# Dimev/grail-rs

Measured on AMD Instinct MI355X. Metric: audio samples/sec (whole node) at 48 kHz, batch=65536 utterances, higher is better.
Workload: dtype f32

## Files before the change

### grail-rs_amd/csrc/api_internal.hpp

```cpp
#pragma once

#include <dlfcn.h>
#include <hip/hip_runtime.h>
#include <rccl/rccl.h>

#include <algorithm>
#include <atomic>
#include <cmath>
#include <condition_variable>
#include <cstdio>
#include <deque>
#include <map>
#include <memory>
#include <mutex>
#include <thread>
#include <cstdlib>
#include <cstring>
#include <new>
#include <string>
#include <type_traits>
#include <unordered_map>
#include <utility>
#include <vector>

#include "../../include/grail_hip.h"
#include "division_window.h"
#include "dyn_plan.h"
#include "fir_plan.h"
#include "iir_plan.h"
#include "kernels.h"
#include "limit_plan.h"
#include "meter_plan.h"
#include "resample_plan.h"


#ifdef GRAIL_FAST_PROF
constexpr size_t TRUNCATED_WORDS = 8 + 64;
#else
constexpr size_t TRUNCATED_WORDS = 4;
#endif

struct Options {
    int64_t fast_option = 0;
    int64_t fast_limit = (int64_t)GRAIL_FAST_SHARPNESS_LIMIT;
    int64_t mid_option = 1;
    int64_t mid_limit = (int64_t)GRAIL_FAST_SHARPNESS_LIMIT_EXACT_COEFFICIENTS;
    int64_t lanes_option = 0;
    int64_t skip_silent_option = 1;
    int64_t pipeline_option = 1;
    int64_t pipe_round32 = 1;
    int64_t pipe_spread = 1;
    int64_t pipe4_max_groups = -1;
    int64_t pipe8_max_groups = -1;
    int64_t scan_option = 1;
    int64_t scan_max_utts = -1;
    int64_t scan_split_max = -1;
    int64_t scan_debug = 0;
    int64_t split_option = 1;
    int64_t split_chunks = 0;
    int64_t split_span = 0;
    int64_t split_ff_permille = 165;
    int64_t split_min_utts = -1;
    int64_t composite_option = 1;
    int64_t row_groups_option = 1;
    int64_t ragged_option = 1;
    int64_t two_waves_option = 1;
    int64_t packed_option = 1;
    int64_t sort_option = 1;
};

struct VoiceInfo {
    bool upper_silent = false, live4_ok = false, scan_ok = false, split_ok = false;
    uint32_t warmup = 0;
};

struct VoiceFacts {
    std::vector<VoiceInfo> voice_info;
    bool voices_upper_silent = false;
    bool voices_live4_ok = false;
    bool voices_scan_ok = false;
    bool voices_split_ok = false;
    uint32_t max_warmup = 0;
    float max_rate = 0.0f;
    float max_dt = 0.0f;
    float max_pitch_jitter = 0.0f;
    double voices_sharpness = INFINITY;
    std::vector<double> voice_sharpness;
};

struct LaunchStats {
    std::string last_kernel = "none";
    int last_formants = 8, last_lanes = 0, last_pipe = 0;
    int last_split = 0;
    int last_fast = 0;
    int last_blocks = 0;
    int last_packed = 0;
    uint64_t slow_steps = 0;
    uint64_t fast_tiles = 0, general_steps = 0;
};

namespace grail {
namespace host {

int fail(int status, const std::string &msg);
int hip_fail(hipError_t e, const char *what);
std::string &last_error();

#define HIP_TRY(expr)                                  \
    do {                                               \
        hipError_t e_ = (expr);                        \
        if (e_ != hipSuccess) return ::grail::host::hip_fail(e_, #expr); \
    } while (0)

template <typename H, hipError_t (*Release)(H)>
class Handle {
public:
    Handle() = default;
    Handle(Handle &&o) noexcept : h_(std::exchange(o.h_, H{})) {}
    Handle &operator=(Handle &&o) noexcept
    {
        if (this != &o) {
            reset();
            h_ = std::exchange(o.h_, H{});
        }
        return *this;
    }
    ~Handle() { reset(); }
    H get() const { return h_; }
    void reset()
    {
        if (h_) (void)Release(h_);
        h_ = H{};
    }
    template <typename Make>
    hipError_t renew(Make make)
    {
        reset();
        const hipError_t e = make(&h_);
        if (e != hipSuccess) h_ = H{};
        return e;
    }

private:
    H h_{};
};

struct Event : Handle<hipEvent_t, hipEventDestroy> {
    hipError_t create(bool timing = false)
    {
        return renew([&](hipEvent_t *ev) { return timing ? hipEventCreate(ev) : hipEventCreateWithFlags(ev, hipEventDisableTiming); });
    }
    operator hipEvent_t() const { return get(); }
};

struct Stream : Handle<hipStream_t, hipStreamDestroy> {
    hipError_t create()
    {
        return renew([](hipStream_t *s) { return hipStreamCreateWithFlags(s, hipStreamNonBlocking); });
    }
    operator hipStream_t() const { return get(); }
};

template <typename T>
class DeviceBuffer {
public:
    T *get() const { return static_cast<T *>(mem_.get()); }
    size_t capacity() const { return mem_.get() ? cap_ : 0; }
    void reset() { mem_.reset(); }
    hipError_t alloc(size_t n)
    {
        cap_ = std::max<size_t>(n, 1);
        return mem_.renew([&](void **p) { return hipMalloc(p, cap_ * sizeof(T)); });
    }
    int reserve(hipStream_t stream, size_t need, size_t want)
    {
        if (capacity() >= std::max<size_t>(need, 1)) return GRAIL_OK;
        if (get()) HIP_TRY(hipStreamSynchronize(stream));
        HIP_TRY(alloc(want));
        return GRAIL_OK;
    }
    int reserve(hipStream_t stream, size_t need) { return reserve(stream, need, need); }

private:
    Handle<void *, hipFree> mem_;
    size_t cap_ = 0;
};

template <typename Tp>
hipError_t upload(DeviceBuffer<Tp> &dst, const void *src, size_t count, hipStream_t stream)
{
    const hipError_t e = dst.alloc(count);
    if (e != hipSuccess || !src || !count) return e;
    return hipMemcpyAsync(dst.get(), src, count * sizeof(Tp), hipMemcpyHostToDevice, stream);
}

struct RowIndex {
    std::vector<uint32_t> host;
    DeviceBuffer<uint32_t> dev;
    hipError_t fill(const uint32_t *given, uint32_t n_rows, bool own_row, hipStream_t stream)
    {
        host.resize(n_rows);
        for (uint32_t u = 0; u < n_rows; ++u) host[u] = given ? given[u] : (own_row ? u : 0u);
        return upload(dev, host.data(), n_rows, stream);
    }
};

class PinnedBuffer {
public:
    void *get() const { return mem_.get(); }
    size_t capacity() const { return mem_.get() ? cap_ : 0; }
    void reset() { mem_.reset(); }
    hipError_t alloc(size_t bytes)
    {
        cap_ = bytes;
        return mem_.renew([&](void **p) { return hipHostMalloc(p, bytes, hipHostMallocDefault); });
    }

private:
    Handle<void *, hipHostFree> mem_;
    size_t cap_ = 0;
};

struct Family {
    int L = 1;
    uint32_t pipe = 0;
    uint32_t live4 = 0;
    bool half = false;
    uint32_t fast = 0;
    int split_k = 0;
    uint32_t split_bounds[SPLIT_MAX_CHUNKS + 1] = {};
    uint32_t split_active = 0;
    bool scan = false;
    uint32_t scan_pipe = 0;
};

struct Block {
    uint32_t rows;
    Family f;
};

struct PlanCache {
    uint64_t key[6] = {};
    std::vector<Block> plan;
};

}
}

struct PlanEnv {
    int cus = 256;
    Options opt;
    VoiceFacts facts;
    uint64_t voices_epoch = 0;
};

struct CtxPart {
    virtual ~CtxPart() = default;
};

struct grail_ctx : PlanEnv {
    int device = 0;
    int device_cus = 256;
    grail::host::Stream stream;
    grail::host::Event ev_start, ev_stop;
    bool have_timing = false;
    uint64_t options_epoch = 0;
    std::vector<grail_voice> voices;
    grail::host::DeviceBuffer<grail::DevVoice> d_voices;
    grail::host::DeviceBuffer<float> d_voice_elems;
    LaunchStats stats;
    grail::host::DeviceBuffer<uint32_t> d_truncated;
    uint32_t seen_counters[4] = {0, 0, 0, 0};
    ncclComm_t comm = nullptr;
    uint32_t comm_rank = 0, comm_world = 1;
    std::unique_ptr<CtxPart> host_pipe;
    std::unique_ptr<CtxPart> mix_state;
    std::unique_ptr<CtxPart> level_state;
    std::unique_ptr<CtxPart> transform_state;
};

struct grail_stream {
    const grail_batch *batch = nullptr;
    grail::host::DeviceBuffer<uint32_t> d_state;
    uint64_t lanes = 0;
    int L = 1;
    bool started = false;
    bool live4 = false, half_capable = false, any_blend = false;
    uint64_t voices_epoch = 0;
    std::unique_ptr<grail_batch> own;
    uint32_t ring_cap = 0;
    grail::host::DeviceBuffer<uint32_t> d_counts;
    grail::host::DeviceBuffer<uint32_t> d_open;
    grail::host::DeviceBuffer<uint32_t> d_consumed;
    std::vector<uint32_t> appended;
    std::vector<uint32_t> consumed;
    std::vector<uint8_t> open;
    std::vector<grail_synthesis_elem> last_elem;
    std::vector<uint8_t> last_has;
    grail::host::DeviceBuffer<grail::DevSeg> d_new;
    grail::host::DeviceBuffer<float> d_new_elems;
    grail::host::DeviceBuffer<uint32_t> d_new_offs;
    grail::host::PinnedBuffer h_stage[2];
    grail::host::Event ev_stage[2];
    bool stage_busy[2] = {false, false};
    int stage_next = 0;
};

struct grail_fir {
    uint32_t n_filters = 0;
    uint32_t tail_max = 0;
    std::vector<double> image;
    std::vector<uint32_t> desc;
    grail::host::DeviceBuffer<double> d_taps;
    grail::host::DeviceBuffer<uint32_t> d_desc;
    uint32_t taps_max = 0;
};

struct ChunkedStream {
    uint32_t n_rows = 0;
    uint32_t units = 0;
    uint32_t ring_cap = 0;
    grail::host::DeviceBuffer<uint64_t> d_state;
    grail::host::DeviceBuffer<float> d_ring;
    std::vector<uint8_t> mark;
    grail::host::DeviceBuffer<uint8_t> d_mark;
    grail::host::Event ev_mark;
};

struct grail_filter_stream : ChunkedStream {
    const grail_fir *set = nullptr;
    grail::host::RowIndex filter;
};

struct grail_resample_stream : ChunkedStream {
    uint32_t up = 0, down = 0, taps = 0;
    std::vector<int32_t> table;
    grail::host::DeviceBuffer<int32_t> d_table;
};

struct grail_limit_stream : ChunkedStream {
    uint32_t group = 1;
    float ceiling = 0.0f;
    uint32_t ell = 0;
};

struct grail_meter_stream : ChunkedStream {
    uint32_t sample_rate = 0, hop = 0;
    uint64_t max_hops = 0;
    double coef[10] = {};
    grail::host::DeviceBuffer<double> d_ledger;
};

struct grail_iir {
    uint32_t n_filters = 0;
    uint32_t bound = 1;
    std::vector<double> image;
    std::vector<uint32_t> sections;
    grail::host::DeviceBuffer<double> d_image;
    grail::host::DeviceBuffer<uint32_t> d_sections;
    std::vector<double> block_image;
    grail::host::DeviceBuffer<double> d_block;
};

struct grail_iir_stream : ChunkedStream {
    const grail_iir *set = nullptr;
    uint32_t tail = 0;
    grail::host::RowIndex filter;
};

struct grail_dyn {
    uint32_t n_curves = 0;
    std::vector<double> image;
    std::vector<double> alpha;
    std::vector<uint32_t> detector;
    grail::host::DeviceBuffer<double> d_image;
    grail::host::DeviceBuffer<double> d_alpha;
    grail::host::DeviceBuffer<uint32_t> d_detector;
};

struct grail_dyn_stream : ChunkedStream {
    const grail_dyn *set = nullptr;
    uint32_t n_keys = 0;
    grail::host::RowIndex curve;
    grail::host::RowIndex key_row;
};

struct BatchFacts {
    uint32_t n_utt = 0;
    uint32_t n_segs = 0;
    uint32_t max_voice_id = 0;
    bool phoneme_mode = true;
    bool any_blend = false;
    bool plain = false;
    float max_seconds = 0.0f;
    float min_length = 0.0f;
    float min_pitch = 0.0f;
    uint64_t len_bound_epoch = 0;
    bool len_bound_known = false;
    double elems_sharpness = 0.0;
    uint32_t elems_warmup = 0;
    uint64_t elems_warmup_epoch = 0;
    bool elems_live4_ok = false;
    bool elems_scan_ok = false;
    std::vector<uint32_t> used_voices;
    std::vector<float> granule_samples;
    std::vector<uint32_t> granule_segs, granule_kinks;
};

struct RowGroup : BatchFacts {
    uint32_t slot0 = 0;
    mutable grail::host::PlanCache plan_cache;
};

struct PackedPerm {
    uint32_t view = 0;
    uint32_t slot0 = 0, rows = 0, per_block = 0, cus = 0;
    uint32_t family = 0;
    grail::host::DeviceBuffer<uint32_t> d_perm;
    double model_ms = 0.0, plain_ms = 0.0;
};

struct grail_batch : BatchFacts {
    grail::host::DeviceBuffer<grail::DevSeg> d_segs;
    grail::host::DeviceBuffer<uint32_t> d_offsets, d_voice_ids, d_seeds;
    grail::host::DeviceBuffer<uint32_t> d_perm;
    std::vector<uint32_t> perm_host;
    grail::host::DeviceBuffer<uint32_t> d_len_bound;
    grail::host::DeviceBuffer<float> d_elems;
    std::vector<RowGroup> groups;
    uint64_t groups_epoch = 0;
    mutable std::mutex lock;
    mutable grail::host::PlanCache plan_cache;
    mutable std::vector<PackedPerm> packed;
};
static_assert(!std::is_copy_constructible_v<grail_batch>, "a batch owns its device arrays: row groups are BatchFacts, not batches");

#include "launch_plan.h"

namespace grail {
namespace host {

int bind(grail_ctx *ctx);
int bind_device(grail_ctx *ctx, const char *who);

void name_voices(BatchFacts &b, const uint32_t *voice_ids, uint32_t n_utt);
bool blend_is_pow2(float blend_length);
int check_offsets(const uint32_t *seg_offsets, uint32_t n_utt, uint32_t *n_segs);
int install_voices(grail_ctx *ctx, const grail_voice *voices, uint32_t n_voices);
int check_ready(grail_ctx *ctx, const grail_batch *batch);

bool live4_ok(const grail_voice &v);
bool live4_elems_ok(const grail_synthesis_elem *elems, size_t n_elems, float jitter_delta_formant_frequency);
bool scan_voice_ok(const grail_voice &v);
bool scan_elems_ok(const grail_synthesis_elem *elems, size_t n_elems, float jitter_delta_formant_frequency);
uint32_t voice_warmup(const grail_voice &v);
uint32_t elems_warmup(const grail_synthesis_elem *elems, size_t n_elems, double jitter_delta_formant_frequency);
double elems_sharpness(const grail_synthesis_elem *elems, size_t n);
double batch_sharpness(const PlanEnv *ctx, const BatchFacts *batch);
int fast_tier_for(const PlanEnv *ctx, const BatchFacts *batch, int arithmetic);
int fast_tier(const PlanEnv *ctx, const BatchFacts *batch);
bool split_grid(uint32_t span, uint32_t warmup, int K, double r, uint32_t *b);

void batch_args(const grail_ctx *ctx, const grail_batch *batch, uint32_t row0, SynthArgs &a);
int synthesize_rows(grail_ctx *ctx, const grail_batch *batch, float *out_dev, int16_t *out_pcm16_dev, uint64_t out_stride,
                    uint32_t *out_len_dev, uint32_t first = 0, uint32_t count = 0, uint32_t family_rows = 0);

void comm_release(grail_ctx *ctx);
int drop_batch(grail_ctx *ctx, grail_batch *batch, int rc);
int level_block_gains(grail_ctx *ctx, int mode, uint32_t sample_rate, const float *rows_dev, uint64_t row_stride,
                      const uint32_t *len_dev, const uint32_t *row_len, uint32_t n_rows, const uint32_t *item_rows,
                      const float *item_level_db, uint32_t n_items, float *gains, uint32_t *n_unleveled,
                      const float *ceiling_db, uint32_t *n_limited);
uint32_t level_table_rate(const grail_ctx *ctx);
int say_segments(const std::vector<grail_voice> &voices, const char *const *texts_utf8, uint32_t n_texts,
                 const uint32_t *voice_ids, std::vector<grail_phoneme_elem> &segs, std::vector<uint32_t> &offs);
int comm_init_all(grail_ctx *const *ctxs, const int *devices, uint32_t n);

}
}
```

### grail-rs_amd/csrc/family_cost.cpp

```cpp
#include "api_internal.hpp"

#include <functional>
#include <queue>

using namespace grail;
using namespace grail::host;

namespace grail {
namespace host {

double batch_span(const PlanEnv *ctx, const BatchFacts *batch, uint64_t out_stride)
{
    double span = std::ceil((double)batch->max_seconds * ctx->facts.max_rate) + 64.0;
    if (!(span >= 64.0)) span = 64.0;
    return std::fmin(span, (double)(out_stride ? out_stride : 1));
}

constexpr double MID_MS_4 = 32.6, MID_MS_8 = 57.2;
static double lane_ms_per_sample(bool fast, bool live4, int L)
{
    static const double exact4[4] = {40.6, 26.9, 16.3, 18.2}, exact8[4] = {77.1, 43.5, 25.8, 15.7};
    static const double fast4[4] = {15.5, 13.6, 12.8, 12.1}, fast8[4] = {23.6, 16.4, 13.3, 12.0};
    const int i = L == 1 ? 0 : L == 2 ? 1 : L == 4 ? 2 : 3;
    return (fast ? (live4 ? fast4 : fast8) : (live4 ? exact4 : exact8))[i] / 96006.0;
// ... 61 lines not shown
    const bool nfa4 = f.live4 != 0;
    const int li = f.L == 1 ? 0 : f.L == 2 ? 1 : f.L == 4 ? 2 : 3;
    if (!f.fast) {
        const double T = (f.L == 1 || (!nfa4 && f.L == 4)) ? 32.0 : 64.0;
        const double tiles = std::fmax(samples / T, 1.0);
        const double event_tiles = tiles * (1.0 - std::exp(-segs / tiles));
        const double runs = f.L == 1 ? 1.0 : f.L == 2 ? (nfa4 ? 0.74 : 0.60) : f.L == 4 ? (nfa4 ? 0.51 : 1.0) : 0.58;
        return samples * lane_ms_per_sample(false, nfa4, f.L) + event_tiles * (nfa4 ? 0.007 : 0.008) * (T / 32.0) * runs +
               (f.L == 1 ? segs * (nfa4 ? 0.0015 : 0.0037) : 0.0);
    }
    static const double m4[4] = {1.16, 1.10, 1.06, 1.02}, c4[4] = {0.00475, 0.0050, 0.00675, 0.00925};
    static const double m8[4] = {1.08, 1.06, 1.04, 1.02}, c8[4] = {0.00775, 0.00675, 0.0070, 0.0095};
    const double events = segs + kinks;
    const double density = events / ((64.0 / (double)f.L) * std::fmax(samples, 1.0));
    const double m = 1.0 + ((nfa4 ? m4 : m8)[li] - 1.0) * std::fmin(1.0, density / 3.0e-4);
    const double rate = f.fast == 2u ? mid_ms_per_sample(nfa4) : lane_ms_per_sample(true, nfa4, f.L);
    return samples * rate * m + events * (nfa4 ? c4 : c8)[li];
}

struct WaveRows {
    double samples = 0.0, segs = 0.0, kinks = 0.0;
};
static WaveRows wave_rows(const BatchFacts *batch, size_t g, size_t per_wave, size_t g1)
{
    WaveRows w;
    for (size_t k = g; k < std::min(g + per_wave, g1); ++k) {
        w.samples = std::fmax(w.samples, (double)batch->granule_samples[k]);
        w.segs += batch->granule_segs[k];
        w.kinks += batch->granule_kinks[k];
    }
    return w;
}
double ragged_wave_cost(const BatchFacts *batch, const Family &f, size_t g, size_t per_wave, size_t g1, double span)
{
    const WaveRows w = wave_rows(batch, g, per_wave, g1);
    return ragged_wave_ms(f, std::fmin(w.samples + 64.0, span), w.segs, w.kinks);
}
static double mean_samples(const BatchFacts *batch, const GranuleRange &r)
{
    double mean = 0.0;
    for (size_t g = r.g0; g < r.g1; ++g) mean += (double)batch->granule_samples[g];
    return mean / (double)(r.g1 - r.g0);
}

static double ragged_scan_cost(const PlanEnv *ctx, const BatchFacts *batch, const Family &f, const GranuleRange &r, uint32_t rows,
                               double span)
{
    return std::fmax(family_cost(ctx, f, rows, std::fmin(mean_samples(batch, r) + 64.0, span)),
                     family_cost(ctx, f, 1u, std::fmin(span, (double)batch->granule_samples[r.g0] + 64.0)));
}

static double ragged_pipe_cost(const PlanEnv *ctx, const BatchFacts *batch, const Family &f, const GranuleRange &r, uint32_t rows,
                               double span)
{
    const size_t g0 = r.g0, g1 = r.g1;
    double longest = std::fmin(span, std::fmax((double)batch->granule_samples[g0], 0.0) + 64.0);
    if (std::ceil((double)rows / (f.live4 ? 16.0 : 8.0)) > (double)ctx->cus)
        longest = 0.55 * longest + 0.45 * std::fmin(longest, mean_samples(batch, r) + 64.0);
    double c = family_cost(ctx, f, rows, longest);
    c *= 1.15;
    double segs = batch->granule_segs[g0];
    if (f.live4 && g0 + 1 < g1) segs += batch->granule_segs[g0 + 1];
    const uint32_t fill = pipe_fill_for(ctx, batch, f, rows);
    if (fill) segs *= (double)fill / (f.live4 ? 16.0 : 8.0);
    const double rounds = std::fmax(longest / 32.0, 1.0);
    const double groups = std::ceil((double)rows / (f.live4 ? 16.0 : 8.0));
    c += 0.011 * rounds * (1.0 - std::exp(-segs / rounds)) * std::ceil(groups / ((f.pipe == 2 ? 1.0 : 2.0) * (double)ctx->cus));
    return c;
}

static double ragged_split_cost(const PlanEnv *ctx, const BatchFacts *batch, const Family &f, const GranuleRange &r, uint32_t rows)
{
    const WaveRows w = wave_rows(batch, r.g0, 8, r.g1);
    const double len = std::fmax((double)batch->granule_samples[r.g0], 64.0), part = (double)f.split_bounds[1] / len;
    Family lane = f;
    lane.split_k = 0;
    lane.L = 1;
    return split_rounds(ctx, f, rows) * (1.2 * ragged_wave_ms(lane, (double)f.split_bounds[1], w.segs * part, w.kinks * part) + 0.12);
}

static double two_wave_cost(const PlanEnv *ctx, const BatchFacts *batch, const Family &f, const GranuleRange &r, double span)
{
    const size_t g0 = r.g0, g1 = r.g1, per_wave = granules_per_wave(f);
    const uint64_t simds = ctx_simds(ctx);
    struct Simd { double t, a, b; };
    auto take = [](Simd &m, const double w) {
        if (m.b < 0.0) m.b = w;
        else if (w <= m.b) m.a = w;
        else { m.a = m.b; m.b = w; }
    };
    double ev_sum = 0.0, lane_samples = 0.0;
    for (size_t g = g0; g < g1; ++g) {
        ev_sum += (double)batch->granule_segs[g] + (double)batch->granule_kinks[g];
        lane_samples += 8.0 * std::fmax((double)batch->granule_samples[g], 1.0);
    }
    const double pace2 = 1.0 / (2.0 * cohabit_gain(f, ev_sum / std::fmax(lane_samples, 1.0)));
    std::vector<Simd> sm(simds, Simd{0.0, -1.0, -1.0});
    auto next_done = [&](const Simd &m) {
        return m.a < 0.0 ? m.t + m.b : m.t + m.a / pace2;
    };
    typedef std::pair<double, size_t> Ev;
    std::priority_queue<Ev, std::vector<Ev>, std::greater<Ev>> done_at;
    const size_t n_waves = (g1 - g0 + per_wave - 1) / per_wave;
    const bool fold = n_waves > simds && n_waves <= 2 * simds;
    size_t g = g0, filled = 0;
    for (; g < g1 && filled < 2 * simds; g += per_wave, ++filled)
        take(sm[filled % simds], ragged_wave_cost(batch, f, fold && filled >= simds ? g0 + (n_waves - 1 - (filled - simds)) * per_wave : g,
                                                  per_wave, g1, span));
    for (size_t i = 0; i < simds; ++i)
        if (sm[i].b >= 0.0) done_at.push(Ev(next_done(sm[i]), i));
    double makespan = 0.0;
    while (!done_at.empty()) {
        const Ev ev = done_at.top();
        done_at.pop();
        Simd &m = sm[ev.second];
        if (m.a < 0.0) {
            m.t += m.b;
            m.b = -1.0;
        } else {
            m.t += m.a / pace2;
            m.b -= m.a;
            m.a = -1.0;
        }
        makespan = std::fmax(makespan, m.t);
        if (g < g1) {
            take(m, ragged_wave_cost(batch, f, g, per_wave, g1, span));
            g += per_wave;
        }
        if (m.b >= 0.0) done_at.push(Ev(next_done(m), ev.second));
    }
    const double waves = std::ceil((double)(g1 - g0) / (double)per_wave);
    const double scale = !f.fast ? (f.L == 2 ? 0.84 : 0.91) : (f.L == 2 && waves > 2.0 * (double)simds ? 1.15 : 1.0);
    return makespan * scale;
}

static double dispatched_cost(const PlanEnv *ctx, const BatchFacts *batch, const Family &f, uint32_t slot0, uint32_t rows, double span)
{
    double plain_ms = 0.0, packed_ms = 0.0;
    const bool packed = packed_launch_order(ctx, batch, f, slot0, rows, span, nullptr, nullptr, &plain_ms, &packed_ms);
    return 0.96 * (packed ? packed_ms : plain_ms);
}

double ragged_cost(const PlanEnv *ctx, const BatchFacts *batch, const Family &f, uint32_t slot0, uint32_t rows, double span)
{
    if (batch->granule_samples.empty() || rows == 0) return family_cost(ctx, f, rows, span);
    const GranuleRange r = granule_range(batch, slot0, rows);
    if (f.scan) return ragged_scan_cost(ctx, batch, f, r, rows, span);
    if (f.pipe) return ragged_pipe_cost(ctx, batch, f, r, rows, span);
    if (f.split_k) return ragged_split_cost(ctx, batch, f, r, rows);
    if (family_cohabits(ctx, f, rows)) return two_wave_cost(ctx, batch, f, r, span);
    return dispatched_cost(ctx, batch, f, slot0, rows, span);
}

}
}
```

### grail-rs_amd/csrc/grail_api.cpp

```cpp
#include "api_internal.hpp"

using namespace grail;
using namespace grail::host;

static_assert(sizeof(grail_synthesis_elem) == 196, "SynthesisElem is 49 x f32");
static_assert(sizeof(grail_phoneme_elem) == sizeof(DevSeg), "PhonemeElem uploads as-is");
static_assert(offsetof(grail_phoneme_elem, phoneme) == offsetof(DevSeg, elem), "layout");
static_assert(offsetof(grail_phoneme_elem, frequency) == offsetof(DevSeg, frequency), "layout");
static_assert(sizeof(grail_voice) == 4 + 2 * 196 + 5 * 4, "Voice layout");
static_assert(GRAIL_UNIQUE_ID_BYTES == NCCL_UNIQUE_ID_BYTES, "unique id size");

namespace grail {
namespace host {

namespace {
thread_local std::string g_last_error;
std::atomic<uint64_t> g_epoch{0};
}

std::string &last_error() { return g_last_error; }

int fail(int status, const std::string &msg)
{
    g_last_error = msg;
// ... 207 lines not shown
    b.used_voices.assign(voice_ids, voice_ids + n_utt);
    std::sort(b.used_voices.begin(), b.used_voices.end());
    b.used_voices.erase(std::unique(b.used_voices.begin(), b.used_voices.end()), b.used_voices.end());
    b.max_voice_id = b.used_voices.back();
}

int upload_common(grail_ctx *ctx, grail_batch *b, const uint32_t *seg_offsets,
                  const uint32_t *voice_ids, const uint32_t *jitter_seeds, uint32_t n_utt)
{
    HIP_TRY(upload(b->d_offsets, seg_offsets, (size_t)n_utt + 1, ctx->stream));
    name_voices(*b, voice_ids, n_utt);
    if (voice_ids) HIP_TRY(upload(b->d_voice_ids, voice_ids, n_utt, ctx->stream));
    if (jitter_seeds) HIP_TRY(upload(b->d_seeds, jitter_seeds, n_utt, ctx->stream));
    b->n_utt = n_utt;
    HIP_TRY(hipStreamSynchronize(ctx->stream));
    return GRAIL_OK;
}

int install_voices(grail_ctx *ctx, const grail_voice *voices, uint32_t n_voices)
{
    if (!voices || n_voices == 0) return fail(GRAIL_ERR_INVALID_ARG, "no voices given");
    std::vector<DevVoice> dv(n_voices);
    std::vector<float> elems((size_t)n_voices * NUM_VOICED * ELEM_FLOATS);
    for (uint32_t v = 0; v < n_voices; ++v) {
        dv[v].sample_rate = voices[v].sample_rate;
        dv[v].jitter_frequency = voices[v].jitter_frequency;
        dv[v].jitter_delta_frequency = voices[v].jitter_delta_frequency;
        dv[v].jitter_delta_formant_frequency = voices[v].jitter_delta_formant_frequency;
        dv[v].jitter_delta_amplitude = voices[v].jitter_delta_amplitude;
        dv[v].elem_base = v * NUM_VOICED;
        dv[v].warmup = voice_warmup(voices[v]);
        dv[v].pad = 0;
        std::memcpy(&elems[(size_t)v * NUM_VOICED * ELEM_FLOATS], voices[v].phonemes,
                    sizeof(grail_synthesis_elem) * NUM_VOICED);
    }
    HIP_TRY(hipStreamSynchronize(ctx->stream));
    ctx->voices.clear();
    HIP_TRY(upload(ctx->d_voices, dv.data(), dv.size(), ctx->stream));
    HIP_TRY(upload(ctx->d_voice_elems, elems.data(), elems.size(), ctx->stream));
    HIP_TRY(hipStreamSynchronize(ctx->stream));
    VoiceFacts facts;
    facts.voices_upper_silent = facts.voices_live4_ok = facts.voices_scan_ok = facts.voices_split_ok = true;
    facts.voices_sharpness = 0.0;
    facts.voice_info.resize(n_voices);
    facts.voice_sharpness.resize(n_voices);
    for (uint32_t v = 0; v < n_voices; ++v) {
        VoiceInfo &vi = facts.voice_info[v];
        vi.upper_silent = true;
        for (int p = 0; p < NUM_VOICED; ++p)
            for (int i = NF / 2; i < NF; ++i) {
                uint32_t bits;
                std::memcpy(&bits, &voices[v].phonemes[p].formant_amp[i], sizeof bits);
                vi.upper_silent = vi.upper_silent && bits == 0u;
            }
        vi.live4_ok = live4_ok(voices[v]);
        vi.scan_ok = scan_voice_ok(voices[v]);
        vi.warmup = dv[v].warmup;
        vi.split_ok = dv[v].warmup != 0u && voices[v].sample_rate > 0.0f && std::isfinite(voices[v].sample_rate);
        facts.voices_upper_silent = facts.voices_upper_silent && vi.upper_silent;
        facts.voices_live4_ok = facts.voices_live4_ok && vi.live4_ok;
        facts.voices_scan_ok = facts.voices_scan_ok && vi.scan_ok;
        facts.voices_split_ok = facts.voices_split_ok && vi.split_ok;
        if (vi.warmup > facts.max_warmup) facts.max_warmup = vi.warmup;
        if (voices[v].sample_rate > facts.max_rate) facts.max_rate = voices[v].sample_rate;
        const float dt = 1.0f / voices[v].sample_rate;
        if (!(dt <= facts.max_dt)) facts.max_dt = dt;
        const float pj = std::fabs(voices[v].jitter_delta_frequency);
        if (!(pj <= facts.max_pitch_jitter)) facts.max_pitch_jitter = pj;
        facts.voice_sharpness[v] = elems_sharpness(voices[v].phonemes, NUM_VOICED);
        facts.voices_sharpness = std::fmax(facts.voices_sharpness, facts.voice_sharpness[v]);
    }
    ctx->voices.assign(voices, voices + n_voices);
    ctx->voices_epoch = ++g_epoch;
    ctx->facts = std::move(facts);
    return GRAIL_OK;
}

int check_ready(grail_ctx *ctx, const grail_batch *batch)
{
    if (!batch) return fail(GRAIL_ERR_INVALID_ARG, "batch is NULL");
    if (ctx->voices.empty() || !ctx->d_voices.get() || !ctx->d_voice_elems.get())
        return fail(GRAIL_ERR_NO_VOICES, "call grail_set_voices first");
    if (batch->max_voice_id >= ctx->voices.size())
        return fail(GRAIL_ERR_INVALID_ARG, "a voice id exceeds the voice table");
    return GRAIL_OK;
}

}
}

extern "C" {

int grail_abi_version(void) { return GRAIL_ABI_VERSION; }

const char *grail_status_string(int status)
{
    switch (status) {
    case GRAIL_OK: return "ok";
    case GRAIL_ERR_INVALID_ARG: return "invalid argument";
    case GRAIL_ERR_NO_DEVICE: return "no usable HIP device (there is no CPU fallback)";
    case GRAIL_ERR_HIP: return "HIP runtime error";
    case GRAIL_ERR_BUFFER_TOO_SMALL: return "an utterance did not end within out_stride samples";
    case GRAIL_ERR_OUT_OF_MEMORY: return "out of device memory";
    case GRAIL_ERR_RCCL: return "RCCL error";
    case GRAIL_ERR_NO_VOICES: return "no voice table set";
    default: return "unknown status";
    }
}

const char *grail_last_error(void) { return g_last_error.c_str(); }

int grail_device_count(int *count)
{
    if (!count) return fail(GRAIL_ERR_INVALID_ARG, "count is NULL");
    *count = 0;
    int n = 0;
    hipError_t e = hipGetDeviceCount(&n);
    if (e != hipSuccess) return hip_fail(e, "hipGetDeviceCount");
    *count = n;
    return GRAIL_OK;
}

int grail_device_pci_bus_id(grail_ctx *ctx, char *out, size_t cap)
{
    if (!ctx || !out || cap < 16) return fail(GRAIL_ERR_INVALID_ARG, "grail_device_pci_bus_id: NULL argument or cap < 16");
    out[0] = 0;
    HIP_TRY(hipDeviceGetPCIBusId(out, (int)cap, ctx->device));
    return GRAIL_OK;
}

int grail_create(int device, grail_ctx **out)
{
    if (!out) return fail(GRAIL_ERR_INVALID_ARG, "out is NULL");
    *out = nullptr;
    int n = 0;
    hipError_t e = hipGetDeviceCount(&n);
    if (e != hipSuccess || n <= 0)
        return fail(GRAIL_ERR_NO_DEVICE,
                    std::string("no HIP device: ") + (e != hipSuccess ? hipGetErrorString(e) : "count 0"));
    if (device < 0 || device >= n) return fail(GRAIL_ERR_NO_DEVICE, "device index out of range");
    HIP_TRY(hipSetDevice(device));
    hipDeviceProp_t prop;
    HIP_TRY(hipGetDeviceProperties(&prop, device));
    if (std::strncmp(prop.gcnArchName, "gfx950", 6) != 0)
        return fail(GRAIL_ERR_NO_DEVICE, std::string("device ") + std::to_string(device) + " is " + prop.gcnArchName +
                                             ": this library holds gfx950 (MI355X) kernels only");
    if (prop.multiProcessorCount <= 0) return fail(GRAIL_ERR_NO_DEVICE, "the device reports no compute units");
    std::unique_ptr<grail_ctx> ctx(new (std::nothrow) grail_ctx());
    if (!ctx) return fail(GRAIL_ERR_OUT_OF_MEMORY, "host allocation failed");
    ctx->device = device;
    ctx->cus = ctx->device_cus = prop.multiProcessorCount;
    hipError_t err;
    if ((err = ctx->stream.create()) != hipSuccess ||
        (err = ctx->ev_start.create(true)) != hipSuccess ||
        (err = ctx->ev_stop.create(true)) != hipSuccess ||
        (err = ctx->d_truncated.alloc(TRUNCATED_WORDS)) != hipSuccess ||
        (err = hipMemsetAsync(ctx->d_truncated.get(), 0, TRUNCATED_WORDS * sizeof(uint32_t), ctx->stream)) != hipSuccess ||
        (err = hipStreamSynchronize(ctx->stream)) != hipSuccess)
        return hip_fail(err, "grail_create");
    *out = ctx.release();
    return GRAIL_OK;
}

int grail_destroy(grail_ctx *ctx)
{
    if (!ctx) return GRAIL_OK;
    (void)hipSetDevice(ctx->device);
    if (ctx->stream) (void)hipStreamSynchronize(ctx->stream);
    comm_release(ctx);
    delete ctx;
    return GRAIL_OK;
}

int grail_set_voices(grail_ctx *ctx, const grail_voice *voices, uint32_t n_voices)
{
    int rc = bind(ctx);
    if (rc) return rc;
    return install_voices(ctx, voices, n_voices);
}

int grail_get_voices(grail_ctx *ctx, grail_voice *voices, uint32_t cap, uint32_t *n_voices)
{
    if (!ctx) return fail(GRAIL_ERR_INVALID_ARG, "ctx is NULL");
    if (n_voices) *n_voices = (uint32_t)ctx->voices.size();
    if (voices)
        for (uint32_t i = 0; i < cap && i < ctx->voices.size(); ++i) voices[i] = ctx->voices[i];
    return GRAIL_OK;
}

uint64_t grail_length_bound(const float *segment_lengths, uint32_t n_segments, float sample_rate)
{
    if (!(sample_rate > 0.0f) || (n_segments && !segment_lengths)) return UINT64_MAX;
    const double dt = (double)(1.0f / sample_rate);
    double samples = 0.0;
    for (uint32_t i = 0; i < n_segments; ++i) {
        if (!std::isfinite(segment_lengths[i])) return UINT64_MAX;
        samples += segment_bound(segment_lengths[i], dt);
    }
    return samples < 1.8e19 ? (uint64_t)samples : UINT64_MAX;
}

int grail_batch_upload(grail_ctx *ctx, const grail_phoneme_elem *segs, const uint32_t *seg_offsets,
                       const uint32_t *voice_ids, const uint32_t *jitter_seeds, uint32_t n_utt,
                       grail_batch **out)
{
    int rc = bind(ctx);
    if (rc) return rc;
    if (!out) return fail(GRAIL_ERR_INVALID_ARG, "out is NULL");
    *out = nullptr;
    uint32_t n_segs = 0;
    if ((rc = check_offsets(seg_offsets, n_utt, &n_segs))) return rc;
    if (n_segs && !segs) return fail(GRAIL_ERR_INVALID_ARG, "segs is NULL");
    for (uint32_t i = 0; i < n_segs; ++i)
        if (segs[i].phoneme < 0 || segs[i].phoneme >= GRAIL_PH_COUNT)
            return fail(GRAIL_ERR_INVALID_ARG, "phoneme discriminant out of range");
    std::unique_ptr<grail_batch> b(new (std::nothrow) grail_batch());
    if (!b) return fail(GRAIL_ERR_OUT_OF_MEMORY, "host allocation failed");
    b->phoneme_mode = true;
    b->n_segs = n_segs;
    const std::vector<RowStats> rows = batch_stats(ctx, b.get(), segs, seg_offsets, n_utt,
                                                   [](float f) { return std::fmin(f, 0.5f); });
    HIP_TRY(upload(b->d_segs, segs, n_segs, ctx->stream));
    if ((rc = upload_common(ctx, b.get(), seg_offsets, voice_ids, jitter_seeds, n_utt)) ||
        (rc = upload_len_bound(ctx, b.get(), rows, n_utt)) || (rc = upload_length_order(ctx, b.get(), rows, n_utt)))
        return rc;
    *out = b.release();
    return GRAIL_OK;
}

int grail_batch_upload_elems(grail_ctx *ctx, const grail_sequence_elem *segs,
                             const uint32_t *seg_offsets, const uint32_t *voice_ids,
                             const uint32_t *jitter_seeds, uint32_t n_utt, grail_batch **out)
{
    int rc = bind(ctx);
    if (rc) return rc;
    if (!out) return fail(GRAIL_ERR_INVALID_ARG, "out is NULL");
    *out = nullptr;
    uint32_t n_segs = 0;
    if ((rc = check_offsets(seg_offsets, n_utt, &n_segs))) return rc;
    if (n_segs && !segs) return fail(GRAIL_ERR_INVALID_ARG, "segs is NULL");
    std::vector<DevSeg> ds(n_segs);
    std::vector<float> elems((size_t)(n_segs ? n_segs : 1) * ELEM_FLOATS);
    for (uint32_t i = 0; i < n_segs; ++i) {
        ds[i].elem = segs[i].has_elem ? (int32_t)i : -1;
        ds[i].length = segs[i].length;
        ds[i].blend_length = segs[i].blend_length;
        ds[i].frequency = segs[i].elem.frequency;
        std::memcpy(&elems[(size_t)i * ELEM_FLOATS], &segs[i].elem, sizeof(grail_synthesis_elem));
    }
    std::unique_ptr<grail_batch> b(new (std::nothrow) grail_batch());
    if (!b) return fail(GRAIL_ERR_OUT_OF_MEMORY, "host allocation failed");
    b->phoneme_mode = false;
    b->n_segs = n_segs;
    const std::vector<RowStats> rows = batch_stats(ctx, b.get(), ds.data(), seg_offsets, n_utt, [](float f) { return f; });
    struct FormantsHash {
        size_t operator()(const float *p) const
        {
            uint64_t h = 0x9E3779B97F4A7C15ull, w;
            for (int i = 0; i < 24; ++i) {
                std::memcpy(&w, p + 1 + 2 * i, sizeof w);
                h = (h ^ w) * 0xFF51AFD7ED558CCDull;
                h ^= h >> 29;
            }
            return (size_t)h;
        }
    };
    struct FormantsEq {
        bool operator()(const float *a, const float *c) const { return std::memcmp(a + 1, c + 1, 48 * sizeof(float)) == 0; }
    };
    std::unordered_map<const float *, uint32_t, FormantsHash, FormantsEq> ids;
    std::vector<grail_synthesis_elem> distinct;
    std::vector<uint32_t> id_of(n_segs, 0xFFFFFFFFu);
    for (uint32_t i = 0; i < n_segs; ++i) {
        if (!segs[i].has_elem) continue;
        const auto it = ids.emplace((const float *)&segs[i].elem, (uint32_t)distinct.size());
        if (it.second) distinct.push_back(segs[i].elem);
        id_of[i] = it.first->second;
    }
    std::unordered_map<uint64_t, double> pair_sharpness;
    for (uint32_t u = 0; u < n_utt; ++u)
        for (uint32_t i = seg_offsets[u]; i < seg_offsets[u + 1]; ++i) {
            if (!segs[i].has_elem) continue;
            const uint32_t a = id_of[i];
            const uint32_t c = (i + 1 < seg_offsets[u + 1] && segs[i + 1].has_elem) ? id_of[i + 1] : a;
            const uint64_t key = ((uint64_t)std::min(a, c) << 32) | std::max(a, c);
            auto it = pair_sharpness.find(key);
            if (it == pair_sharpness.end()) {
                const grail_synthesis_elem pair[2] = {distinct[a], distinct[c]};
                it = pair_sharpness.emplace(key, elems_sharpness(pair, a == c ? 1 : 2)).first;
            }
            b->elems_sharpness = std::fmax(b->elems_sharpness, it->second);
        }
    HIP_TRY(upload(b->d_segs, ds.data(), n_segs, ctx->stream));
    HIP_TRY(upload(b->d_elems, elems.data(), elems.size(), ctx->stream));
    if ((rc = upload_common(ctx, b.get(), seg_offsets, voice_ids, jitter_seeds, n_utt)) ||
        (rc = upload_len_bound(ctx, b.get(), rows, n_utt)) || (rc = upload_length_order(ctx, b.get(), rows, n_utt)))
        return rc;
    if (!ctx->voices.empty() && b->max_voice_id < ctx->voices.size()) {
        double jd = 0.0;
        bool rates_ok = true;
        for (const uint32_t v : b->used_voices) {
            jd = std::fmax(jd, std::fabs((double)ctx->voices[v].jitter_delta_formant_frequency));
            rates_ok = rates_ok && ctx->voices[v].sample_rate > 0.0f && std::isfinite(ctx->voices[v].sample_rate);
        }
        bool voices4 = true;
        for (const uint32_t v : b->used_voices) {
            grail_voice scalars = ctx->voices[v];
            for (int ph = 0; ph < NUM_VOICED; ++ph) grail_elem_silent(&scalars.phonemes[ph]);
            voices4 = voices4 && live4_ok(scalars);
        }
        b->elems_live4_ok = voices4 && live4_elems_ok(distinct.data(), distinct.size(), (float)jd);
        b->elems_warmup = rates_ok ? elems_warmup(distinct.data(), distinct.size(), jd) : 0u;
        float max_pitch = 0.0f;
        for (uint32_t i = 0; i < n_segs; ++i) max_pitch = std::fmax(max_pitch, segs[i].elem.frequency);
        b->elems_scan_ok = rates_ok && max_pitch <= 0.5f && scan_elems_ok(distinct.data(), distinct.size(), (float)jd);
        b->elems_warmup_epoch = ctx->voices_epoch;
        for (RowGroup &g : b->groups) {
            g.elems_warmup = b->elems_warmup;
            g.elems_warmup_epoch = b->elems_warmup_epoch;
            g.elems_live4_ok = b->elems_live4_ok;
            g.elems_scan_ok = b->elems_scan_ok;
// ... 203 lines not shown
```

### grail-rs_amd/csrc/synthesize.cpp

```cpp
#include "api_internal.hpp"

using namespace grail;
using namespace grail::host;

namespace grail {
namespace host {

struct View {
    const BatchFacts *facts;
    PlanCache *cache;
    uint32_t id, slot0;
};

void batch_args(const grail_ctx *ctx, const grail_batch *batch, uint32_t row0, SynthArgs &a)
{
    a.segs = batch->d_segs.get();
    a.seg_offsets = batch->d_offsets.get() + row0;
    a.voice_ids = batch->d_voice_ids.get() ? batch->d_voice_ids.get() + row0 : nullptr;
    a.seeds = batch->d_seeds.get() ? batch->d_seeds.get() + row0 : nullptr;
    a.elems = batch->phoneme_mode ? ctx->d_voice_elems.get() : batch->d_elems.get();
    a.voices = ctx->d_voices.get();
    a.truncated = ctx->d_truncated.get();
    a.n_voices = (uint32_t)ctx->voices.size();
    a.phoneme_mode = batch->phoneme_mode ? 1u : 0u;
    a.skip_silent = ctx->opt.skip_silent_option ? 1u : 0u;
}

static const uint32_t *packed_perm_of(grail_ctx *ctx, const grail_batch *root, const View &view, const Family &f,
                                      uint64_t out_stride, uint32_t slot0, uint32_t count, int *rc)
{
    *rc = GRAIL_OK;
    if (!ctx->opt.packed_option || root->perm_host.size() < (size_t)slot0 + count) return nullptr;
    const uint32_t family = (uint32_t)f.L | f.fast << 8 | f.live4 << 16;
    std::lock_guard<std::mutex> hold(root->lock);
    for (const PackedPerm &pp : root->packed)
        if (pp.view == view.id && pp.slot0 == slot0 && pp.rows == count && pp.family == family && pp.cus == (uint32_t)ctx->cus)
            return pp.d_perm.get();
    if (root->packed.size() >= 8) return nullptr;
    PackedPerm pp;
    pp.view = view.id;
    pp.slot0 = slot0;
    pp.rows = count;
    pp.family = family;
    pp.cus = (uint32_t)ctx->cus;
    std::vector<uint32_t> order;
    if (packed_launch_order(ctx, view.facts, f, slot0 - view.slot0, count, batch_span(ctx, view.facts, out_stride), &order,
                            &pp.per_block, &pp.plain_ms, &pp.model_ms)) {
        std::vector<uint32_t> perm(count);
        const uint32_t *src = root->perm_host.data() + slot0;
        size_t at = 0;
        for (const uint32_t b : order) {
            const size_t lo = (size_t)b * pp.per_block, hi = std::min<size_t>(lo + pp.per_block, count);
            for (size_t i = lo; i < hi; ++i) perm[at++] = src[i];
        }
        hipError_t e = at == count ? upload(pp.d_perm, perm.data(), count, ctx->stream) : hipErrorInvalidValue;
        if (e == hipSuccess) e = hipStreamSynchronize(ctx->stream);
        if (e != hipSuccess) {
            *rc = hip_fail(e, "packed launch order");
            return nullptr;
        }
    }
    root->packed.push_back(std::move(pp));
    return root->packed.back().d_perm.get();
}

static int launch_block(grail_ctx *ctx, const grail_batch *root, const View &view, const Family &f, float *out_dev,
                        int16_t *out_pcm16_dev, uint64_t out_stride, uint32_t *out_len_dev, uint32_t first, uint32_t slot0,
                        uint32_t count, bool use_perm)
{
    const BatchFacts *batch = view.facts;
    SynthArgs a{};
    const uint32_t row0 = use_perm ? 0u : first + slot0;
    const uint64_t out_shift = use_perm ? 0ull : (uint64_t)slot0 * out_stride;
    batch_args(ctx, root, row0, a);
    a.out_pcm16 = out_pcm16_dev ? out_pcm16_dev + out_shift : nullptr;
    a.perm = use_perm ? root->d_perm.get() + slot0 : nullptr;
    if (use_perm) {
        int rc = GRAIL_OK;
        const uint32_t *packed = packed_perm_of(ctx, root, view, f, out_stride, slot0, count, &rc);
        if (rc) return rc;
        if (packed) {
            a.perm = packed;
            ++ctx->stats.last_packed;
        }
    }
    a.out = out_dev ? out_dev + out_shift : nullptr;
    a.out_len = out_len_dev ? out_len_dev + (use_perm ? 0u : slot0) : nullptr;
    a.out_stride = out_stride;
    a.cap = out_stride;
    a.n_utt = count;
    a.half_capable = batch_half_capable(ctx, batch) ? 1u : 0u;
    a.any_blend = batch->any_blend ? 1u : 0u;
    a.live4 = f.live4;
    a.fast = f.fast;
    a.cohabit = family_cohabits(ctx, f, count) ? 1u : 0u;
    a.len_bound = root->d_len_bound.get() && batch->len_bound_epoch == ctx->voices_epoch ? root->d_len_bound.get() + row0 : nullptr;
    a.pipe_fill = pipe_fill_for(ctx, batch, f, count);
    a.fold_from = 0u;
    if (a.cohabit) {
        const WorkgroupShape wg = workgroup_shape(f);
        const uint32_t blocks = (count + wg.rows - 1u) / wg.rows, round = (uint32_t)ctx_simds(ctx) / wg.waves;
        if (blocks > round && blocks <= 2u * round) a.fold_from = round;
    }
    a.pipe = f.pipe;
    hipError_t e;
    if (f.scan) {
        a.resume = (uint32_t)ctx->opt.scan_debug;
        a.pipe = f.scan_pipe;
        e = launch_scan(a, ctx->stream);
        ctx->stats.last_kernel = a.live4 ? (a.pipe ? "scan_kernel<pairs=2,SPLIT,FAST>" : "scan_kernel<pairs=2,FAST>")
                                   : (a.pipe ? "scan_kernel<pairs=4,SPLIT,FAST>" : "scan_kernel<pairs=4,FAST>");
    } else {
        if (f.split_k) {
            a.split_chunks = (uint32_t)f.split_k;
            a.split_warmup = batch->phoneme_mode ? 0u : batch->elems_warmup;
            std::memcpy(a.split_bounds, f.split_bounds, sizeof a.split_bounds);
        }
        e = launch_synth(a, f.L, ctx->stream);
        ctx->stats.last_kernel = last_kernel_name();
    }
    if (e != hipSuccess) return hip_fail(e, "synth kernel launch");
    return GRAIL_OK;
}

static void record_plan(LaunchStats &st, const Family &f0, size_t n_blocks)
{
    st.last_split = f0.split_k;
    st.last_formants = f0.live4 ? 4 : 8;
    st.last_lanes = f0.scan ? 0 : f0.L;
    st.last_pipe = f0.pipe && !f0.scan ? 1 : 0;
    st.last_packed = 0;
    st.last_fast = 0;
    st.last_blocks = (int)n_blocks;
}

int synthesize_rows(grail_ctx *ctx, const grail_batch *batch, float *out_dev,
                           int16_t *out_pcm16_dev, uint64_t out_stride, uint32_t *out_len_dev,
                           uint32_t first, uint32_t count, uint32_t family_rows)
{
    int rc = bind(ctx);
    if (rc) return rc;
    if ((rc = check_ready(ctx, batch))) return rc;
    if (batch->n_utt == 0) return GRAIL_OK;
    if (!out_dev && !out_pcm16_dev && out_stride) return fail(GRAIL_ERR_INVALID_ARG, "out_dev is NULL");
    if (first > batch->n_utt || count > batch->n_utt - first) return fail(GRAIL_ERR_INVALID_ARG, "row range");
    if (count == 0) count = batch->n_utt - first;
    if (count == 0) return GRAIL_OK;
    const bool use_perm = first == 0 && count == batch->n_utt && batch->d_perm.get();
    auto plan_of = [&](const View &view, const uint32_t rows) {
        const BatchFacts *facts = view.facts;
        std::vector<Block> plan;
        const uint64_t key[6] = {rows, out_stride, family_rows, ctx->options_epoch, ctx->voices_epoch,
                                 (uint64_t)(uintptr_t)ctx ^ (facts->phoneme_mode ? 0ull : (uint64_t)(facts->elems_sharpness * 1024.0))};
        {
            std::lock_guard<std::mutex> hold(batch->lock);
            if (!view.cache->plan.empty() && std::memcmp(view.cache->key, key, sizeof key) == 0) return view.cache->plan;
        }
        const bool single = family_rows != 0 || !ctx->opt.composite_option || ctx->opt.lanes_option || ctx->opt.split_chunks >= 2;
        if (single) {
            Family f;
            choose_family(ctx, facts, out_stride, family_rows > rows ? family_rows : rows, f);
            plan.push_back(Block{rows, f});
        } else {
            plan_blocks(ctx, facts, out_stride, rows, batch_span(ctx, facts, out_stride), plan);
            if (use_perm && view.slot0 == 0) ragged_plan(ctx, facts, out_stride, rows, plan);
        }
        {
            std::lock_guard<std::mutex> hold(batch->lock);
            std::memcpy(view.cache->key, key, sizeof key);
            view.cache->plan = plan;
        }
        return plan;
    };
    struct Part {
        View view;
        Block block;
    };
    const View whole{batch, &batch->plan_cache, 0u, 0u};
    std::vector<Part> plan;
    for (const Block &b : plan_of(whole, count)) plan.push_back(Part{whole, b});
    if (use_perm && family_rows == 0 && ctx->opt.row_groups_option && batch->groups.size() == 2 && batch->groups_epoch == ctx->voices_epoch) {
        auto cost_of = [&](const std::vector<Part> &parts) {
            double c = 0.0;
            uint32_t at = 0, of = 0xFFFFFFFFu;
            for (const Part &p : parts) {
                if (p.view.id != of) at = 0;
                of = p.view.id;
                c += ragged_cost(ctx, p.view.facts, p.block.f, at, p.block.rows, batch_span(ctx, p.view.facts, out_stride)) + 0.05;
                at += p.block.rows;
            }
            return c;
        };
        std::vector<Part> grouped;
        for (uint32_t g = 0; g < 2; ++g) {
            const RowGroup &group = batch->groups[g];
            const View view{&group, &group.plan_cache, 1u + g, group.slot0};
            for (const Block &b : plan_of(view, group.n_utt)) grouped.push_back(Part{view, b});
        }
        if (ctx->opt.row_groups_option == 2 || cost_of(grouped) < cost_of(plan)) plan.swap(grouped);
    }
    size_t main_block = 0;
    for (size_t i = 1; i < plan.size(); ++i)
        if (plan[i].block.rows > plan[main_block].block.rows) main_block = i;
    const Family f0 = plan[main_block].block.f;
    record_plan(ctx->stats, f0, plan.size());
    HIP_TRY(hipEventRecord(ctx->ev_start, ctx->stream));
    uint32_t slot0 = 0;
    std::string first_kernel;
    for (size_t i = 0; i < plan.size(); ++i) {
        const Block &b = plan[i].block;
        rc = launch_block(ctx, batch, plan[i].view, b.f, out_dev, out_pcm16_dev, out_stride, out_len_dev, first, slot0, b.rows, use_perm);
        if (rc) return rc;
        if (i == main_block) first_kernel = ctx->stats.last_kernel;
        if ((int)b.f.fast > ctx->stats.last_fast) ctx->stats.last_fast = (int)b.f.fast;
        slot0 += b.rows;
    }
    ctx->stats.last_kernel = first_kernel;
    HIP_TRY(hipEventRecord(ctx->ev_stop, ctx->stream));
    ctx->have_timing = true;
    return GRAIL_OK;
}


}
}

extern "C" {

int grail_batch_synthesize_async(grail_ctx *ctx, const grail_batch *batch, float *out_dev,
                                 uint64_t out_stride, uint32_t *out_len_dev)
{
    return synthesize_rows(ctx, batch, out_dev, nullptr, out_stride, out_len_dev);
}

int grail_batch_synthesize_pcm16_async(grail_ctx *ctx, const grail_batch *batch, int16_t *out_dev,
                                       uint64_t out_stride, uint32_t *out_len_dev)
{
    return synthesize_rows(ctx, batch, nullptr, out_dev, out_stride, out_len_dev);
}

}
```

Measured before the change: 157.2 billion.

## Run independent plan blocks concurrently on side streams when resources fit

Result: no change. 157.2 billion (median of 2 runs) (-0.0%).

```diff
diff --git a/grail-rs_amd/csrc/api_internal.hpp b/grail-rs_amd/csrc/api_internal.hpp
--- a/grail-rs_amd/csrc/api_internal.hpp
+++ b/grail-rs_amd/csrc/api_internal.hpp
@@ -40,7 +40,17 @@
 constexpr size_t TRUNCATED_WORDS = 4;
 #endif
 
+#ifndef GRAIL_CONCURRENT_BLOCKS
+#define GRAIL_CONCURRENT_BLOCKS 1
+#endif
+inline int64_t concurrent_blocks_default()
+{
+    const char *e = std::getenv("GRAIL_CONCURRENT_BLOCKS");
+    return e && *e ? (*e != '0' ? 1 : 0) : (GRAIL_CONCURRENT_BLOCKS ? 1 : 0);
+}
+
 struct Options {
+    int64_t concurrent_option = concurrent_blocks_default();
     int64_t fast_option = 0;
     int64_t fast_limit = (int64_t)GRAIL_FAST_SHARPNESS_LIMIT;
     int64_t mid_option = 1;
@@ -262,6 +272,8 @@
     int device = 0;
     int device_cus = 256;
     grail::host::Stream stream;
+    grail::host::Stream side[2];
+    grail::host::Event ev_side[2];
     grail::host::Event ev_start, ev_stop;
     bool have_timing = false;
     uint64_t options_epoch = 0;
@@ -440,6 +452,13 @@
 namespace grail {
 namespace host {
 
+double block_chain_ms(const PlanEnv *ctx, const BatchFacts *batch, const Family &f, uint32_t slot0, double span);
+struct KernelFootprint {
+    uint32_t regs, lds, waves;
+};
+KernelFootprint family_footprint(const Family &f, bool two);
+bool blocks_run_concurrently(const PlanEnv *ctx, const std::vector<Block> &blocks);
+
 int bind(grail_ctx *ctx);
 int bind_device(grail_ctx *ctx, const char *who);
 
diff --git a/grail-rs_amd/csrc/family_cost.cpp b/grail-rs_amd/csrc/family_cost.cpp
--- a/grail-rs_amd/csrc/family_cost.cpp
+++ b/grail-rs_amd/csrc/family_cost.cpp
@@ -237,5 +237,49 @@
     return dispatched_cost(ctx, batch, f, slot0, rows, span);
 }
 
-}
-}
+double block_chain_ms(const PlanEnv *ctx, const BatchFacts *batch, const Family &f, uint32_t slot0, double span)
+{
+    double longest = span;
+    if (!batch->granule_samples.empty())
+        longest = std::fmin(span, (double)batch->granule_samples[granule_range(batch, slot0, 1u).g0] + 64.0);
+    Family unit = f;
+    unit.split_active = 0;
+    return family_cost(ctx, unit, 1u, longest);
+}
+
+KernelFootprint family_footprint(const Family &f, bool two)
+{
+    auto up8 = [](uint32_t r) { return (r + 7u) / 8u * 8u; };
+    if (f.scan) return {128u, f.scan_pipe ? 26228u : 17508u, f.scan_pipe ? 3u : 2u};
+    if (f.pipe) return f.pipe == 2 ? KernelFootprint{up8(296u), 131968u, 4u} : KernelFootprint{up8(252u), 74624u, 4u};
+    const bool nfa4 = f.live4 != 0;
+    if (f.L == 1) {
+        if (!f.fast) return {up8(nfa4 ? 274u : 496u), 8832u, 1u};
+        return {up8(f.fast == 2u ? (nfa4 ? 322u : 477u) : (nfa4 ? 350u : 482u)), 17152u, 1u};
+    }
+    if (f.L == 2) return {up8(two ? (f.fast ? 235u : 213u) : (f.fast ? (nfa4 ? 364u : 384u) : (nfa4 ? 344u : 384u))), 8704u, 1u};
+    if (f.L == 4) {
+        if (two) return {up8(f.fast ? (nfa4 ? 230u : 202u) : (nfa4 ? 255u : 201u)), 66048u, 4u};
+        return {up8(f.fast ? (nfa4 ? 360u : 352u) : (nfa4 ? 384u : 328u)), 66048u, 4u};
+    }
+    return {up8(two ? 235u : (f.fast ? 364u : 384u)), 65792u, 4u};
+}
+
+bool blocks_run_concurrently(const PlanEnv *ctx, const std::vector<Block> &blocks)
+{
+    if (!ctx->opt.concurrent_option || blocks.size() < 2) return false;
+    size_t main_block = 0;
+    uint32_t regs = 0, lds = 0;
+    for (size_t i = 0; i < blocks.size(); ++i) {
+        const Block &b = blocks[i];
+        if (b.rows > blocks[main_block].rows) main_block = i;
+        const bool two = family_cohabits(ctx, b.f, b.rows);
+        const KernelFootprint fp = family_footprint(b.f, two);
+        regs += fp.regs * (two ? 2u : 1u);
+        lds += fp.lds * (two ? 2u : 1u) * (fp.waves == 1u ? 4u : 1u);
+    }
+    return blocks[main_block].f.fast != 0u && regs <= 512u && lds <= 160u * 1024u;
+}
+
+}
+}
diff --git a/grail-rs_amd/csrc/grail_api.cpp b/grail-rs_amd/csrc/grail_api.cpp
--- a/grail-rs_amd/csrc/grail_api.cpp
+++ b/grail-rs_amd/csrc/grail_api.cpp
@@ -383,6 +383,8 @@
     ctx->cus = ctx->device_cus = prop.multiProcessorCount;
     hipError_t err;
     if ((err = ctx->stream.create()) != hipSuccess ||
+        (err = ctx->side[0].create()) != hipSuccess || (err = ctx->side[1].create()) != hipSuccess ||
+        (err = ctx->ev_side[0].create()) != hipSuccess || (err = ctx->ev_side[1].create()) != hipSuccess ||
         (err = ctx->ev_start.create(true)) != hipSuccess ||
         (err = ctx->ev_stop.create(true)) != hipSuccess ||
         (err = ctx->d_truncated.alloc(TRUNCATED_WORDS)) != hipSuccess ||
@@ -398,6 +400,8 @@
     if (!ctx) return GRAIL_OK;
     (void)hipSetDevice(ctx->device);
     if (ctx->stream) (void)hipStreamSynchronize(ctx->stream);
+    for (const Stream &s : ctx->side)
+        if (s) (void)hipStreamSynchronize(s);
     comm_release(ctx);
     delete ctx;
     return GRAIL_OK;
diff --git a/grail-rs_amd/csrc/synthesize.cpp b/grail-rs_amd/csrc/synthesize.cpp
--- a/grail-rs_amd/csrc/synthesize.cpp
+++ b/grail-rs_amd/csrc/synthesize.cpp
@@ -66,7 +66,7 @@
 
 static int launch_block(grail_ctx *ctx, const grail_batch *root, const View &view, const Family &f, float *out_dev,
                         int16_t *out_pcm16_dev, uint64_t out_stride, uint32_t *out_len_dev, uint32_t first, uint32_t slot0,
-                        uint32_t count, bool use_perm)
+                        uint32_t count, bool use_perm, hipStream_t stream)
 {
     const BatchFacts *batch = view.facts;
     SynthArgs a{};
@@ -107,7 +107,7 @@
     if (f.scan) {
         a.resume = (uint32_t)ctx->opt.scan_debug;
         a.pipe = f.scan_pipe;
-        e = launch_scan(a, ctx->stream);
+        e = launch_scan(a, stream);
         ctx->stats.last_kernel = a.live4 ? (a.pipe ? "scan_kernel<pairs=2,SPLIT,FAST>" : "scan_kernel<pairs=2,FAST>")
                                    : (a.pipe ? "scan_kernel<pairs=4,SPLIT,FAST>" : "scan_kernel<pairs=4,FAST>");
     } else {
@@ -116,7 +116,7 @@
             a.split_warmup = batch->phoneme_mode ? 0u : batch->elems_warmup;
             std::memcpy(a.split_bounds, f.split_bounds, sizeof a.split_bounds);
         }
-        e = launch_synth(a, f.L, ctx->stream);
+        e = launch_synth(a, f.L, stream);
         ctx->stats.last_kernel = last_kernel_name();
     }
     if (e != hipSuccess) return hip_fail(e, "synth kernel launch");
@@ -204,16 +204,55 @@
         if (plan[i].block.rows > plan[main_block].block.rows) main_block = i;
     const Family f0 = plan[main_block].block.f;
     record_plan(ctx->stats, f0, plan.size());
-    HIP_TRY(hipEventRecord(ctx->ev_start, ctx->stream));
-    uint32_t slot0 = 0;
     std::string first_kernel;
-    for (size_t i = 0; i < plan.size(); ++i) {
+    auto launch = [&](const size_t i, const uint32_t slot0, hipStream_t stream) {
         const Block &b = plan[i].block;
-        rc = launch_block(ctx, batch, plan[i].view, b.f, out_dev, out_pcm16_dev, out_stride, out_len_dev, first, slot0, b.rows, use_perm);
-        if (rc) return rc;
+        const int r = launch_block(ctx, batch, plan[i].view, b.f, out_dev, out_pcm16_dev, out_stride, out_len_dev, first, slot0, b.rows,
+                                   use_perm, stream);
+        if (r) return r;
         if (i == main_block) first_kernel = ctx->stats.last_kernel;
         if ((int)b.f.fast > ctx->stats.last_fast) ctx->stats.last_fast = (int)b.f.fast;
-        slot0 += b.rows;
+        return (int)GRAIL_OK;
+    };
+    std::vector<Block> blocks;
+    for (const Part &p : plan) blocks.push_back(p.block);
+    if (!blocks_run_concurrently(ctx, blocks)) {
+        HIP_TRY(hipEventRecord(ctx->ev_start, ctx->stream));
+        uint32_t slot0 = 0;
+        for (size_t i = 0; i < plan.size(); ++i) {
+            if ((rc = launch(i, slot0, ctx->stream))) return rc;
+            slot0 += plan[i].block.rows;
+        }
+    } else {
+        struct Job {
+            size_t i;
+            uint32_t slot0;
+            double chain;
+        };
+        std::vector<Job> jobs;
+        uint32_t slot0 = 0;
+        for (size_t i = 0; i < plan.size(); ++i) {
+            const Part &p = plan[i];
+            const double span = batch_span(ctx, p.view.facts, out_stride);
+            jobs.push_back(Job{i, slot0, block_chain_ms(ctx, p.view.facts, p.block.f, use_perm ? slot0 - p.view.slot0 : 0u, span)});
+            if (use_perm) {
+                (void)packed_perm_of(ctx, batch, p.view, p.block.f, out_stride, slot0, p.block.rows, &rc);
+                if (rc) return rc;
+            }
+            slot0 += p.block.rows;
+        }
+        std::stable_sort(jobs.begin(), jobs.end(), [](const Job &x, const Job &y) { return x.chain > y.chain; });
+        const size_t n_side = std::min<size_t>(2, jobs.size() - 1);
+        auto lane = [&](const size_t k) -> hipStream_t { return k % (n_side + 1) == 0 ? ctx->stream.get() : ctx->side[k % (n_side + 1) - 1].get(); };
+        HIP_TRY(hipEventRecord(ctx->ev_start, ctx->stream));
+        for (size_t s = 0; s < n_side; ++s) HIP_TRY(hipStreamWaitEvent(ctx->side[s], ctx->ev_start, 0));
+        for (size_t k = 0; k < jobs.size() && !rc; ++k) rc = launch(jobs[k].i, jobs[k].slot0, lane(k));
+        for (size_t s = 0; s < n_side; ++s) {
+            hipError_t e = hipEventRecord(ctx->ev_side[s], ctx->side[s]);
+            if (e == hipSuccess) e = hipStreamWaitEvent(ctx->stream, ctx->ev_side[s], 0);
+            if (e != hipSuccess && !rc) rc = hip_fail(e, "joining the side streams");
+        }
+        if (rc) return rc;
     }
     ctx->stats.last_kernel = first_kernel;
     HIP_TRY(hipEventRecord(ctx->ev_stop, ctx->stream));
```
